# lh3/minigraph

Hardware: NVIDIA H100
Metric: mapped Gbp/s (-cx lr) (higher is better)
Workload: dtype int64/u8 (fp32 chain penalties, bit-exact)

## Files before the change

### include/mgb200.h

```cpp
#ifndef MGB200_H
#define MGB200_H

#include <stdint.h>
#include <stddef.h>

#ifdef __cplusplus
extern "C" {
#endif

#ifndef __GFA_H__
#define __GFA_H__
typedef struct {
	uint64_t v_lv;
	uint32_t w;
	int32_t rank;
	int32_t ov, ow;
	uint64_t link_id:61, strong:1, del:1, comp:1;
} gfa_arc_t;

typedef struct { uint32_t m_aux, l_aux; uint8_t *aux; } gfa_aux_t;

typedef struct gfa_utg_s gfa_utg_t;

typedef struct {
// ... 145 lines not shown
	int64_t n_jobs_side;
	int64_t n_slots;
	double t_pack_ms, t_asm_ms;
	int64_t n_jobs;
	int64_t n_jobs_mid, n_jobs_big;
	int64_t n_reads, n_bases;
	int64_t n_seeds;
	int64_t n_anchors_out;
	int64_t n_chains_out;
	int64_t n_minimizers;
	int64_t out_bytes;
	int64_t n_launches;
	int64_t n_retry;
	uint64_t arena_peak;
	double t_kernel_ms[10];
	uint64_t prof[32];
	double t_lab_ms;
	int64_t n_lab_new;
	int64_t n_lab_big;
	int64_t h2d_bytes;
	double w_gpu_wait_ms;
	double w_slot_wait_ms, w_upload_ms, w_pass_ms, w_redo_ms, w_download_ms;
} mgb_stats_t;

int mgb_test_wfa(const char *ts, int tl, const char *qs, int ql, int64_t max_iter, int step, uint32_t *cigar, int cap, int *score);

#define MGB_TEST_TIER2_CONT 4
int mgb_test_wfa_tier(int tier, int n, const char *ts, const int64_t *t_off, const int32_t *tl, const char *qs, const int64_t *q_off,
					  const int32_t *ql, int64_t *out, uint32_t *cigar, int cap);

int mgb_test_gwfa(const mg_idx_t *gi, int mode, int n, const char *q, const int64_t *q_off, const int32_t *ql, const uint32_t *v0,
// ... 34 lines not shown
```

### minigraph_b200/capi.py

```python
import ctypes as C
import os

MG_M_RMQ = 0x8000
MG_M_CIGAR = 0x4000000
MG_M_PRINT_2ND = 0x2000


class mg128_t(C.Structure):
    _fields_ = [("x", C.c_uint64), ("y", C.c_uint64)]


class mg_idxopt_t(C.Structure):
    _fields_ = [("w", C.c_int), ("k", C.c_int), ("bucket_bits", C.c_int)]


class mg_mapopt_t(C.Structure):
    _fields_ = [
        ("flag", C.c_uint64), ("mini_batch_size", C.c_int64), ("seed", C.c_int), ("max_qlen", C.c_int),
        ("pe_ori", C.c_int), ("occ_max1", C.c_int), ("occ_max1_cap", C.c_int), ("occ_max1_frac", C.c_float),
        ("bw", C.c_int), ("bw_long", C.c_int), ("rmq_size_cap", C.c_int), ("rmq_rescue_size", C.c_int),
        ("rmq_rescue_ratio", C.c_float), ("max_gap_pre", C.c_int), ("max_gap", C.c_int), ("max_gap_ref", C.c_int),
        ("max_frag_len", C.c_int), ("div", C.c_float), ("chn_pen_gap", C.c_float), ("chn_pen_skip", C.c_float),
        ("max_lc_skip", C.c_int), ("max_lc_iter", C.c_int), ("max_gc_skip", C.c_int), ("min_lc_cnt", C.c_int),
        ("min_lc_score", C.c_int), ("min_gc_cnt", C.c_int), ("min_gc_score", C.c_int), ("gdp_max_ed", C.c_int),
# ... 49 lines not shown

class gfa_t(C.Structure):
    _fields_ = [("m_seg", C.c_uint32), ("n_seg", C.c_uint32), ("max_rank", C.c_uint32), ("seg", C.POINTER(gfa_seg_t)),
                ("h_names", C.c_void_p), ("m_sseq", C.c_uint32), ("n_sseq", C.c_uint32),
                ("sseq", C.POINTER(gfa_sseq_t)), ("h_snames", C.c_void_p), ("m_arc", C.c_uint64),
                ("n_arc", C.c_uint64), ("arc", C.c_void_p), ("link_aux", C.c_void_p), ("idx", C.POINTER(C.c_uint64))]


class mgb_stats_t(C.Structure):
    _fields_ = [("t_h2d_ms", C.c_double), ("t_seed_ms", C.c_double), ("t_chain_ms", C.c_double),
                ("t_align_ms", C.c_double), ("t_d2h_ms", C.c_double), ("t_host_ms", C.c_double),
                ("t_wfa_ms", C.c_double), ("t_finish_ms", C.c_double), ("t_dev_span_ms", C.c_double), ("skip1_len", C.c_int64), ("skip2_len", C.c_int64), ("n_jobs_side", C.c_int64), ("n_slots", C.c_int64), ("t_pack_ms", C.c_double), ("t_asm_ms", C.c_double),
                ("n_jobs", C.c_int64), ("n_jobs_mid", C.c_int64), ("n_jobs_big", C.c_int64),
                ("n_reads", C.c_int64), ("n_bases", C.c_int64), ("n_seeds", C.c_int64), ("n_anchors_out", C.c_int64),
                ("n_chains_out", C.c_int64), ("n_minimizers", C.c_int64), ("out_bytes", C.c_int64),
                ("n_launches", C.c_int64), ("n_retry", C.c_int64), ("arena_peak", C.c_uint64), ("t_kernel_ms", C.c_double * 10), ("prof", C.c_uint64 * 32), ("t_lab_ms", C.c_double), ("n_lab_new", C.c_int64), ("n_lab_big", C.c_int64), ("h2d_bytes", C.c_int64),
                ("w_gpu_wait_ms", C.c_double), ("w_slot_wait_ms", C.c_double), ("w_upload_ms", C.c_double), ("w_pass_ms", C.c_double), ("w_redo_ms", C.c_double), ("w_download_ms", C.c_double)]


class mgb_reads_t(C.Structure):
    _fields_ = [("n_reads", C.c_int64), ("n_bases", C.c_int64), ("name", C.POINTER(C.c_char_p)), ("seq", C.POINTER(C.c_char_p)),
                ("len", C.POINTER(C.c_int)), ("block", C.c_void_p)]


KERNEL_NAMES = ["k_seed", "k_chain", "k_gchain", "k_index_sketch", "k_wfa_small", "k_finish", "k_wfa_mid", "k_wfa_big", "k_gwfa", "k_gchain_gen"]
PROF_NAMES = ["wfa_fast_cyc", "wfa_fast_n", "wfa_slow_cyc", "wfa_slow_n", "wfa_max_cyc", "wfa_cells", "wfa_tb_cyc", "gc_dp_cyc", "gc_gen_cyc",
              "gc_post_cyc", "gc_plan_cyc", "fin_cigar_cyc", "fin_ds_cyc", "seed_sketch_cyc", "seed_match_cyc", "seed_sort_cyc", "chain_dp_cyc",
              "chain_onchip_n", "chain_rmq_cyc", "chain_post_cyc", "wfa_mid_cyc", "wfa_mid_n", "gc_gwfa_cyc", "gc_bridge_shortk_cyc", "gc_extra_sort_cyc", "gwfa_max_cyc", "gc_dp_max_cyc", "wfa_handoff_cells", "wfa_handoff_n", "lab_cyc", "lab_n"]
WFA_TIER2_CONT = 4
LCHAIN_DP, LCHAIN_RMQ, LCHAIN_RESCUE = 0, 1, 2
LCHAIN_PATH_DP, LCHAIN_PATH_RMQ_W, LCHAIN_PATH_RMQ_TIE, LCHAIN_PATH_RMQ_CAP = 0, 1, 2, 3


class mgb_lchain_opt_t(C.Structure):
    _fields_ = [(k, C.c_int32) for k in ("max_dist_x", "max_dist_y", "bw", "max_skip", "max_iter", "min_cnt", "min_sc")] + \
               [("pen_gap", C.c_float), ("pen_skip", C.c_float)] + \
               [(k, C.c_int32) for k in ("is_cdna", "n_seg", "max_dist_inner", "cap_rmq_size")]


def bind_mapping_api(lib):
    lib.mg_index.restype = C.POINTER(mg_idx_t)
    lib.mg_index.argtypes = [C.POINTER(gfa_t), C.POINTER(mg_idxopt_t), C.c_int, C.POINTER(mg_mapopt_t)]
    lib.mg_idx_destroy.restype = None
# ... 86 lines not shown
```

### minigraph_b200/csrc/mgb_engine.cu

```cuda
#include <stdio.h>
#include <stdlib.h>
#include <string.h>
#include <math.h>
#include <vector>
#include <algorithm>
#include <string>
#include <chrono>
#include <thread>
#include <mutex>
#include <condition_variable>
#include <functional>
#include <unordered_map>
#include "mgb_hostpool.h"

#include "../../include/mgb200.h"
#include "mgb_galign.cuh"
#include "mgb_gaf.cuh"

#ifndef MGB_HOSTSIM
#include <cuda_runtime.h>
#include "mgb_index.cuh"
#endif

using namespace mgb;
// ... 460 lines not shown
#endif
		}
}
#ifndef MGB_HOSTSIM
__global__ void __launch_bounds__(256) k_unpack(UnpackArgs U)
{
	const int lane = threadIdx.x & 31, warp = (int)((blockIdx.x * blockDim.x + threadIdx.x) >> 5), n_warp = (int)((gridDim.x * blockDim.x) >> 5);
	for (int r = warp; r < U.n_reads; r += n_warp) {
		if (U.pk_off[r] == ~0ULL) continue;
		const int64_t nw = ((int64_t)U.seq_len[r] + 31) >> 5;
		for (int64_t wd = lane; wd < nw; wd += 32) unpack_word(U, r, wd);
	}
}
#endif

struct Mail { Pool pools[16]; unsigned int jobq_n[2], lab_n[2]; unsigned long long prof[32]; unsigned int tier_hist[128]; unsigned long long arena_peak; };
struct MailSrc { const Pool *pools; const unsigned int *jobq_n, *lab_n; const unsigned long long *prof; const unsigned int *tier_hist; const uint64_t *peak; int n_workers; };
#ifndef MGB_HOSTSIM
__global__ void k_mail(MailSrc m, Mail *out)
{
	const int t = threadIdx.x;
	if (t < 16) out->pools[t] = m.pools[t];
	if (t < 2) out->jobq_n[t] = m.jobq_n[t], out->lab_n[t] = m.lab_n? m.lab_n[t] : 0;
	out->prof[t] = m.prof[t];
	for (int i = t; i < 128; i += 32) out->tier_hist[i] = m.tier_hist[i];
	unsigned long long pk = 0;
	for (int i = t; i < m.n_workers; i += 32) pk = m.peak[i] > pk? m.peak[i] : pk;
	for (int o = 16; o > 0; o >>= 1) { const unsigned long long y = __shfl_xor_sync(0xffffffffu, pk, o); pk = y > pk? y : pk; }
	if (t == 0) out->arena_peak = pk;
	__threadfence_system();
}
#endif
MG_HD inline void job_counts(const Pool *pools, int i_gjobs, int i_jobs, unsigned int gjobs_done, unsigned int jobs_done, unsigned int *cnt)
{
	const Pool &pg = pools[i_gjobs], &pj = pools[i_jobs];
	cnt[0] = (unsigned int)((pg.used < pg.cap? pg.used : pg.cap) / sizeof(GwfaJob)) - gjobs_done;
	cnt[1] = (unsigned int)((pj.used < pj.cap? pj.used : pj.cap) / sizeof(WfaJob)) - jobs_done;
}
#ifndef MGB_HOSTSIM
// ... 1189 lines not shown
				if (b1 > b0) memcpy(hout + b0, P.packed + b0, b1 - b0);
#endif
			}
			tm_d2h.stop();
			S.out_bytes = (int64_t)out_bytes;
		}
		if (done) break;
		for (int i = 0; i < N_POOLS; ++i) if (hp[i].used > cap[i]) cap[i] = (hp[i].used * 3 / 2 + 4095) & ~(uint64_t)4095;
		if (attempt == 7) { set_error("output pools kept overflowing"); rc_final = -2; }
	}
	S.t_h2d_ms = tm_h2d.ms(), S.t_seed_ms = tm_seed.ms(), S.t_chain_ms = tm_chain.ms(), S.t_align_ms = tm_align.ms();
	S.t_wfa_ms = tm_wfa.ms(), S.t_finish_ms = tm_fin.ms();
	for (int i = 0; i < 10; ++i) S.t_kernel_ms[i] = tm_k[i].ms();
	S.t_lab_ms = tm_lab.ms();
	S.arena_peak = mail->arena_peak;
	for (int i = 0; i < 32; ++i) S.prof[i] = (uint64_t)mail->prof[i];
	{
		const unsigned int *h = mail->tier_hist;
		int32_t t1 = INT32_MAX;
		for (int b = 0; b < 32 && t1 == INT32_MAX; ++b) { unsigned int in = h[b * 4 + 1], out = h[b * 4 + 2] + h[b * 4 + 3]; if (in + out >= 8 && in < out) t1 = b * 16; }
		unsigned int tot = 0;
		for (int i = 0; i < 128; ++i) tot += h[i];
		if (tot >= 64) { std::lock_guard<std::mutex> lock(M->big_mutex); M->skip1_len = t1; }
		S.skip1_len = L_skip1, S.skip2_len = INT32_MAX;
	}
	if (rc_final < 0) return rc_final;

	double t_asm0 = now_ms();
	S.w_download_ms = t_asm0 - t_host0 - S.w_upload_ms - S.w_pass_ms - S.w_redo_ms - S.w_gpu_wait_ms;
	int first_bad = -1;
	for (int i = 0; i < n_reads; ++i) {
// ... 650 lines not shown
```

### minigraph_b200/csrc/mgb_galign.cuh

```cuda
#pragma once
#include "mgb_pipeline.cuh"
#include "mgb_gchain.cuh"
#include "mgb_wfa_tiers.cuh"
#if defined(MGB_HOSTSIM)
#include <stdio.h>
#include <stdlib.h>
#endif

namespace mgb {

MG_HD inline int cigar_append1(Arena &A, AVec<uint64_t> &c, int32_t op, int32_t len)
{
	if (c.n > 0 && (int32_t)(c.a[c.n - 1] & 0xf) == op) c.a[c.n - 1] += (uint64_t)(int64_t)len << 4;
	else {
		uint64_t x = (uint64_t)(int64_t)len << 4 | (uint64_t)op;
		MGB_TRY(avec_push(A, c, x));
	}
	return 0;
}

MG_HD inline int cigar_append(Arena &A, AVec<uint64_t> &c, int32_t n_cigar, const uint32_t *cigar)
{
	if (n_cigar == 0) return 0;
	MGB_TRY(cigar_append1(A, c, (int32_t)(cigar[0] & 0xf), (int32_t)(cigar[0] >> 4)));
// ... 86 lines not shown
	unsigned long long pt0 = prof_clock();
	int rc;
	int64_t cont_cells = 0;
	if (tier == 1) rc = wfa_smem<WfTier1::W_, WfTier1::MAXLEN_, WfTier1::TBCAP_>(A, smem, tl, tseq, ql, qs, &rst, lane);
	else if (tier == 2 && !t2_long) rc = wfa_smem<WfTier2::W_, WfTier2::MAXLEN_, WfTier2::TBCAP_, true>(A, smem, tl, tseq, ql, qs, &rst, lane, &cont_cells);
	else if (tier == 2) rc = wfa_ring_exact(A, tl, tseq, ql, qs, &rst, lane);
	else rc = wfa_exact(A, tl, tseq, ql, qs, 100000000LL, &rst, lane);
	if (rc < 0) return rc;
	if (lane == 0) {
		unsigned long long dt = prof_clock() - pt0;
		int slot = tier == 1? PROF_WFA_FAST_CYC : tier == 2? PROF_WFA_MID_CYC : PROF_WFA_SLOW_CYC;
		prof_add(c, slot, dt), prof_add(c, slot + 1, 1);
		prof_max(c, PROF_WFA_MAX_CYC, dt << 16 | (unsigned long long)(mlen < 65535? mlen : 65535));
		if (rc == 0) prof_add(c, PROF_WFA_CELLS, (unsigned long long)rst.n_iter);
		if (cont_cells > 0) prof_add(c, PROF_WFA_HANDOFF_N, 1), prof_add(c, PROF_WFA_HANDOFF_CELLS, (unsigned long long)cont_cells);
		if (rc == 0 && explore && c.tier_hist) {
			unsigned int *h = &c.tier_hist[(mlen >> 4 < 31? mlen >> 4 : 31) * 4 + tier];
#if MGB_ON_DEVICE
			atomicAdd(h, 1u);
#else
			++*h;
#endif
		}
	}
	if (rc == 1) {
		if (lane == 0) {
			unsigned int at;
#if MGB_ON_DEVICE
			at = atomicAdd(&c.jobq_n[tier - 1], 1u);
#else
// ... 635 lines not shown
```

### minigraph_b200/csrc/mgb_pipeline.cuh

```cuda
#pragma once
#include "mgb_model.cuh"
#include "mgb_seed.cuh"
#include "mgb_lchain.cuh"
#include "mgb_gclabel.cuh"
#include "mgb_tma.cuh"

namespace mgb {

struct PipeCtx {
	GraphDev g;
	IndexDev ix;
	MapOptDev opt;
	BatchDev b;
	ReadMeta *meta;
	Pool *pool_anchor;     u128 *anchor;
	Pool *pool_minipos;    int32_t *minipos;
	Pool *pool_lchain;     LChain *lchain;
	Pool *pool_out;        char *out;
	Pool *pool_plan;       uint64_t *plan;
	Pool *pool_jobs;       struct WfaJob *jobs;
	Pool *pool_cig;        uint32_t *cig;
	int32_t *jobq[2];      unsigned int *jobq_n;
	Pool *pool_gstate;     char *gstate;
	Pool *pool_gjobs;      struct GwfaJob *gjobs;
	Pool *pool_walk;       int32_t *walk;
	int32_t *rescue_list;  unsigned int *rescue_n;
	LabTab lab;
	unsigned int *next_read;
	unsigned long long *prof;
	int32_t skip1_len;
	unsigned int *tier_hist;
};

enum { PROF_WFA_FAST_CYC = 0, PROF_WFA_FAST_N, PROF_WFA_SLOW_CYC, PROF_WFA_SLOW_N, PROF_WFA_MAX_CYC, PROF_WFA_CELLS, PROF_WFA_TB_CYC,
	   PROF_GC_DP_CYC, PROF_GC_GEN_CYC, PROF_GC_POST_CYC, PROF_GC_PLAN_CYC, PROF_FIN_CIGAR_CYC, PROF_FIN_DS_CYC, PROF_SEED_SKETCH_CYC,
	   PROF_SEED_MATCH_CYC, PROF_SEED_SORT_CYC, PROF_CHAIN_DP_CYC, PROF_CHAIN_BT_CYC, PROF_CHAIN_RMQ_CYC, PROF_CHAIN_POST_CYC, PROF_WFA_MID_CYC, PROF_WFA_MID_N, PROF_GC_GWFA_CYC, PROF_GC_SHORTK_CYC, PROF_GC_EXTRA_CYC, PROF_GWFA_MAX_CYC, PROF_GC_DP_MAX_CYC, PROF_WFA_HANDOFF_CELLS, PROF_WFA_HANDOFF_N, PROF_LAB_CYC, PROF_LAB_N, PROF_N = 32 };

MG_HD inline unsigned long long prof_clock()
{
#if MGB_ON_DEVICE
	return (unsigned long long)clock64();
#else
	return 0;
#endif
}
#if defined(__CUDACC__)
MG_D inline unsigned long long *prof_block() { __shared__ unsigned long long s_prof[PROF_N]; return s_prof; }
MG_D inline bool prof_is_max(int slot) { return slot == PROF_WFA_MAX_CYC || slot == PROF_GWFA_MAX_CYC || slot == PROF_GC_DP_MAX_CYC; }
MG_D inline void prof_block_begin() { if (threadIdx.x < PROF_N) prof_block()[threadIdx.x] = 0; __syncthreads(); }
MG_D inline void prof_block_end(unsigned long long *prof)
{
	__syncthreads();
	if (prof && threadIdx.x < PROF_N) {
		const unsigned long long v = prof_block()[threadIdx.x];
		if (v) { if (prof_is_max((int)threadIdx.x)) atomicMax(&prof[threadIdx.x], v); else atomicAdd(&prof[threadIdx.x], v); }
	}
}
#endif
MG_HD inline void prof_add(const PipeCtx &c, int slot, unsigned long long v)
{
#if MGB_ON_DEVICE
	if (c.prof) atomicAdd(&prof_block()[slot], v);
#else
	if (c.prof) c.prof[slot] += v;
#endif
}
MG_HD inline void prof_max(const PipeCtx &c, int slot, unsigned long long v)
{
#if MGB_ON_DEVICE
	if (c.prof) atomicMax(&prof_block()[slot], v);
// ... 325 lines not shown
```

### minigraph_b200/csrc/mgb_wfa.cuh

```cuda
#pragma once
#include "mgb_common.cuh"

namespace mgb {

static const int32_t WF_NEG_INF = -0x40000000;
static const int WF_X = 4, WF_O1 = 4, WF_E1 = 2, WF_O2 = 15, WF_E2 = 1;
static const int WF_MAX_PEN = 16;
static const int WF_NSLICE = WF_MAX_PEN + 1;
static const int WF_PAD = WF_MAX_PEN + 1;
static const int WF_SEQ_PAD = 16;

#define MGB_WF_MAX(a, b) ((a) >= (b)? (a) : (b))

struct WfResult {
	int32_t s;
	int32_t n_cigar;
	int64_t n_iter;
	uint32_t *cigar;
};


MG_HD inline void wf_stage_seq(char *dst, const char *src, int32_t len, uint8_t sentinel, int lane)
{
	for (int32_t i = lane; i < len; i += MGB_W) dst[i] = src[i];
	for (int32_t i = len + lane; i < len + WF_SEQ_PAD; i += MGB_W) dst[i] = (char)sentinel;
}

MG_HD inline uint32_t wf_ld32u(const char *base, int32_t pos)
{
	const uint32_t *w = (const uint32_t*)base;
	uint32_t lo = w[pos >> 2], hi = w[(pos >> 2) + 1];
	int sh = (pos & 3) << 3;
#if MGB_ON_DEVICE
// ... 21 lines not shown
template<typename TB>
MG_HD inline int wf_traceback(const TB &tb, int32_t n_scores, int32_t tl, const char *ts, int32_t ql, const char *qs, int32_t last_state,
							  uint32_t *cig_store, int64_t max_cigar, int32_t *n_cigar, int64_t *first)
{
	int32_t i = ql - 1, k = tl - 1, s = n_scores - 1, last = last_state;
	int64_t w = max_cigar;
	int32_t cur_op = -1, cur_len = 0;
#define MGB_CIG_PUSH(op_, len_) do { \
		if (cur_op == (op_)) cur_len += (len_); \
		else { \
			if (cur_op >= 0) { if (w <= 0) return MGB_E_INTERNAL; cig_store[--w] = (uint32_t)cur_len << 4 | (uint32_t)cur_op; } \
			cur_op = (op_), cur_len = (len_); \
		} \
	} while (0)
	while (i >= 0 && k >= 0) {
		int32_t k0 = k, x, state, ext;
		if (last == 0) {
			while (i >= 0 && k >= 0 && qs[i] == ts[k]) --i, --k;
			if (k0 - k > 0) MGB_CIG_PUSH(7, k0 - k);
			if (i < 0 || k < 0) break;
		}
		if (s < 0) return MGB_E_INTERNAL;
		x = tb.get(s, i - k);
		if (x < 0) return MGB_E_INTERNAL;
		state = last == 0? x & 7 : last;
		ext = state > 0? x >> (state + 2) & 1 : 0;
		if (state == 0) { MGB_CIG_PUSH(8, 1); --i, --k, s -= WF_X; }
		else if (state == 1) { MGB_CIG_PUSH(1, 1); --i, s -= ext? WF_E1 : WF_O1 + WF_E1; }
		else if (state == 3) { MGB_CIG_PUSH(1, 1); --i, s -= ext? WF_E2 : WF_O2 + WF_E2; }
		else if (state == 2) { MGB_CIG_PUSH(2, 1); --k, s -= ext? WF_E1 : WF_O1 + WF_E1; }
		else if (state == 4) { MGB_CIG_PUSH(2, 1); --k, s -= ext? WF_E2 : WF_O2 + WF_E2; }
		else return MGB_E_INTERNAL;
		last = state > 0 && ext? state : 0;
	}
	if (i >= 0) MGB_CIG_PUSH(1, i + 1);
	else if (k >= 0) MGB_CIG_PUSH(2, k + 1);
	if (cur_op >= 0) { if (w <= 0) return MGB_E_INTERNAL; cig_store[--w] = (uint32_t)cur_len << 4 | (uint32_t)cur_op; }
#undef MGB_CIG_PUSH
// ... 18 lines not shown

template<int W>
MG_HD inline int32_t wfs_col(int32_t d) { return (d + (1 << 20)) & (W - 1); }

struct WfTbSmem {
	const int32_t *row; const uint8_t *x; int32_t n_rows, used;
	MG_HD int32_t get(int32_t s, int32_t d) const
	{
		int32_t lo = row[2 * s], off = row[2 * s + 1];
		int32_t end = s + 1 < n_rows? row[2 * s + 3] : used;
		int32_t j = d - lo;
		return (j < 0 || off + j >= end)? -1 : (int32_t)x[off + j];
	}
};

struct WfTbRow { int32_t lo, hi; uint8_t *x; };
struct WfTbArena {
	const WfTbRow *row;
	MG_HD int32_t get(int32_t s, int32_t d) const
	{
		int32_t j = d - row[s].lo;
		return (j < 0 || j > row[s].hi - row[s].lo)? -1 : (int32_t)row[s].x[j];
	}
};



#define MGB_NL_SYNC(nl) do { if ((nl) > 1) warp_sync(); } while (0)

struct WfSlice {
	int32_t lo, hi;
	int32_t *H, *E1, *F1, *E2, *F2;
};

struct WfState {
	WfSlice sl[WF_NSLICE];
	int32_t *mem;
// ... 154 lines not shown
			wf.lo = wf.hi = seg[sid++].d;
		}
		lo = wf.lo > -tl? wf.lo - 1 : -tl;
		hi = wf.hi < ql? wf.hi + 1 : ql;
		{
			const WfSlice &ft = wf_stripe_add(wf, lo, hi, lane, nl);
			const WfSlice &fx = wf_stripe_get(wf, WF_X);
			const WfSlice &fo1 = wf_stripe_get(wf, WF_O1 + WF_E1);
			const WfSlice &fo2 = wf_stripe_get(wf, WF_O2 + WF_E2);
			const WfSlice &fe1 = wf_stripe_get(wf, WF_E1);
			const WfSlice &fe2 = wf_stripe_get(wf, WF_E2);
			if (nl > 1) MGB_TRY(avec_reserve_w(A, rows, rows.n + 1, lane));
			else MGB_TRY(avec_reserve(A, rows, rows.n + 1));
			uint8_t *x;
			MGB_ALLOC(A, x, uint8_t, hi - lo + 1);
			if (lane == 0) rows.a[rows.n].lo = lo, rows.a[rows.n].hi = hi, rows.a[rows.n].x = x;
			++rows.n;
			uint8_t *ax = x - lo;
			for (int32_t dd = lo + lane; dd <= hi; dd += nl)
				ax[dd] = wf_cell(dd, ft.H, ft.E1, ft.F1, ft.E2, ft.F2, fx.H, fo1.H, fo2.H, fe1.E1, fe1.F1, fe2.E2, fe2.F2);
			MGB_NL_SYNC(nl);
			if (ft.H[lo] >= -1 || ft.E1[lo] >= -1 || ft.F1[lo] >= -1 || ft.E2[lo] >= -1 || ft.F2[lo] >= -1) wf.lo = lo;
			if (ft.H[hi] >= -1 || ft.E1[hi] >= -1 || ft.F1[hi] >= -1 || ft.E2[hi] >= -1 || ft.F2[hi] >= -1) wf.hi = hi;
		}
		if ((wf.s & 0xff) == 0) MGB_TRY(wf_stripe_shrink(wf, tl, ql));
		r->n_iter += hi - lo + 1;
		if (max_iter > 0 && r->n_iter > max_iter) { stopped = 1; break; }
	}
	r->s = stopped? -1 : wf.s;
	if (!stopped) {
		int rc = 0;
// ... 396 lines not shown
```

### minigraph_b200/csrc/mgb_wfa_tiers.cuh

```cuda
#pragma once
#include "mgb_wfa.cuh"

namespace mgb {

#if MGB_ON_DEVICE
MG_D inline uint32_t warp_or_u32(uint32_t x) { return __reduce_or_sync(0xffffffffu, x); }
#elif defined(MGB_SIM_LANES)
inline uint32_t warp_or_u32(uint32_t x) { uint64_t o[32]; sim::exchange(x, o, 15); uint32_t r = 0; for (int i = 0; i < MGB_W; ++i) r |= (uint32_t)o[i]; return r; }
#else
inline uint32_t warp_or_u32(uint32_t x) { return x; }
#endif

#define MGB_OPAQUE(x) asm("" : "+r"(x))

MG_HD inline int32_t wf2_ld(const void *base, int32_t off)
{
	int32_t v = *(const wf_cell_t*)((const char*)base + off);
	MGB_OPAQUE(v);
	return v;
}

#define MGB_WF_CELL_LOAD(S, d_) \
	int32_t h##S, e1##S, e2##S, f1##S, f2##S; \
	uint8_t xz##S; \
// ... 58 lines not shown
	return sc < 0? MGB_WF_RG(1, 0) : sc == 0? MGB_WF_RG(0, 0) : MGB_WF_RG(rows[sc - 1].lo, rows[sc - 1].hi);
}

template<int W>
MG_HD inline int wfa_smem_continue(Arena &A, uint64_t mark, const wf_cell_t *sm, int32_t tl, const char *ts, int32_t ql, const char *qs, WfResult *r,
								   uint32_t *cig_store, int64_t max_cigar, int lane, WfRing &R);

template<int W, int MAXLEN, int TBCAP, bool CONT = false>
MG_HD inline int wfa_smem(Arena &A, int32_t *smem, int32_t tl, const char *ts_g, int32_t ql, const char *qs_g, WfResult *r, int lane, int64_t *cont_cells = 0)
{
	static_assert(!CONT || TBCAP == 0, "the arena ring continues from traceback rows in the arena");
	typedef WfSmemLayout<W, MAXLEN, TBCAP, 17> LY;
	const int HS = 17;
	if (tl > MAXLEN || ql > MAXLEN) return 1;
	if (MAXLEN > 16000) return 1;
	uint64_t mark = A.top;
	wf_cell_t *H = (wf_cell_t*)smem, *E1 = H + HS * W, *F1 = E1 + 3 * W, *E2 = F1 + 3 * W, *F2 = E2 + 2 * W;
	char *ts = (char*)(smem + LY::N_INTS), *qs = ts + LY::SEQ_BYTES;
	int32_t *tb_row = (int32_t*)(qs + LY::SEQ_BYTES);
	uint8_t *tb_x = (uint8_t*)tb_row + LY::TB_ROW_BYTES;
	{
		const uint32_t two = (uint32_t)(uint16_t)(wf_cell_t)WF_NEG_INF16 * 0x10001u;
		uint32_t *cells = (uint32_t*)smem;
		for (int32_t i = lane; i < LY::N_INTS; i += MGB_W) cells[i] = two;
	}
	wf_stage_seq(ts, ts_g, tl, 0xfe, lane);
	wf_stage_seq(qs, qs_g, ql, 0xff, lane);
	r->s = -1, r->n_cigar = 0, r->n_iter = 0, r->cigar = 0;
	uint32_t *cig_store;
	const int64_t max_cigar = (int64_t)tl + ql + 2;
	MGB_ALLOC(A, cig_store, uint32_t, max_cigar);
	uint64_t mark_keep = A.top;
	AVec<WfTbRow> rows;
	avec_init(rows);
	if (TBCAP == 0) MGB_TRY(avec_reserve_w(A, rows, 256, lane));
	int32_t n_rows = 0, tb_used = 0;
	int32_t wlo = 0, whi = 0, last_state = 0, s = 0;
	int64_t n_iter = 0;
	int hs = 0, m3 = 0, m2 = 0;
	const int32_t d_corner = ql - tl;
	int hit = 0, hit_noext = 0;
	warp_sync();
	if (lane == 0) {
		int32_t k0 = -1, k = -1;
		if (!(k0 >= tl || k0 >= ql)) {
			k = wf_extend(ts, qs, k0, 0);
			if (k == tl - 1 && k == ql - 1) hit = 1, hit_noext = (k == k0), k = k0;
		}
		H[wfs_col<W>(0)] = (wf_cell_t)k;
	}
	{
		const uint32_t vb = warp_or_u32((hit? 1u : 0u) | (hit_noext? 2u : 0u));
		hit = vb & 1, hit_noext = vb >> 1 & 1;
	}
	warp_sync();
	for (;;) {
		if (hit) {
			if (hit_noext) {
				int32_t x;
				if (TBCAP > 0) { WfTbSmem t; t.row = tb_row, t.x = tb_x, t.n_rows = n_rows, t.used = tb_used; x = t.get(n_rows - 1, ql - tl); }
				else { WfTbArena t; t.row = rows.a; x = t.get(n_rows - 1, ql - tl); }
				last_state = x & 7;
			}
			break;
		}
		const int32_t lo = wlo > -tl? wlo - 1 : -tl;
		const int32_t hi = whi < ql? whi + 1 : ql;
		const int32_t width = hi - lo + 1;
		if (width + 2 > W || s + 1 >= 255 || (TBCAP > 0 && tb_used + width > TBCAP)) {
			if (CONT && s < 240) {
				WfRing R;
				R.rows = rows, R.n_rows = n_rows, R.wlo = wlo, R.whi = whi, R.s = s, R.hs = hs, R.m3 = m3, R.m2 = m2, R.n_iter = n_iter;
				const int rc = wfa_smem_continue<W>(A, mark_keep, H, tl, ts, ql, qs, r, cig_store, max_cigar, lane, R);
				if (rc < 0) { A.top = mark; return rc; }
				if (r->s < 0) { A.top = mark; return MGB_E_INTERNAL; }
				*cont_cells = r->n_iter - n_iter;
				return 0;
			}
			A.top = mark;
			return 1;
		}
		const int32_t ns = s + 1;
		const int nhs = hs + 1 == 17? 0 : hs + 1, n3 = m3 + 1 == 3? 0 : m3 + 1, n2 = m2 ^ 1;
		uint8_t *ax;
		if (TBCAP > 0) {
			if (lane == 0) tb_row[2 * n_rows] = lo, tb_row[2 * n_rows + 1] = tb_used;
			ax = tb_x + tb_used - lo;
			tb_used += width;
		} else {
			uint8_t *x;
			MGB_ALLOC(A, x, uint8_t, width);
			if (lane == 0) rows.a[n_rows].lo = lo, rows.a[n_rows].hi = hi, rows.a[n_rows].x = x;
			rows.n = n_rows + 1;
			ax = x - lo;
		}
		++n_rows;
		const int r4 = nhs >= WF_X? nhs - WF_X : nhs - WF_X + 17, r6 = nhs >= WF_O1 + WF_E1? nhs - (WF_O1 + WF_E1) : nhs - (WF_O1 + WF_E1) + 17;
		const int r16 = nhs >= WF_O2 + WF_E2? nhs - (WF_O2 + WF_E2) : nhs - (WF_O2 + WF_E2) + 17;
		const int e1slot = n3 >= 2? n3 - 2 : n3 + 1;
		int32_t bHx = r4 * W * 2, bHo1 = r6 * W * 2, bHo2 = r16 * W * 2, bE1 = e1slot * W * 2, bE2 = m2 * W * 2, bnH = nhs * W * 2, bn3 = n3 * W * 2, bn2 = n2 * W * 2;
		MGB_OPAQUE(bHx); MGB_OPAQUE(bHo1); MGB_OPAQUE(bHo2); MGB_OPAQUE(bE1); MGB_OPAQUE(bE2); MGB_OPAQUE(bnH); MGB_OPAQUE(bn3); MGB_OPAQUE(bn2);
		const int32_t colmask2 = 2 * W - 1;
		uint32_t vote = 0;
		for (int32_t d = lo + lane; d <= hi; d += MGB_W) {
			MGB_WF_CELL_LOAD(A, d)
			MGB_WF_CELL_FINISH(A, d)
		}
		vote = warp_or_u32(vote);
		if (vote & 1) wlo = lo;
		if (vote & 2) whi = hi;
		hit = vote >> 2 & 1, hit_noext = vote >> 3 & 1;
		s = ns, hs = nhs, m3 = n3, m2 = n2;
		n_iter += width;
		warp_sync();
	}
	r->n_iter = n_iter;
	r->s = s;
	{
		int rc = 0;
		int32_t n_cig = 0;
		int64_t first = 0;
		if (lane == 0) {
			if (TBCAP > 0) { WfTbSmem t; t.row = tb_row, t.x = tb_x, t.n_rows = n_rows, t.used = tb_used; rc = wf_traceback(t, n_rows, tl, ts, ql, qs, last_state, cig_store, max_cigar, &n_cig, &first); }
			else { WfTbArena t; t.row = rows.a; rc = wf_traceback(t, n_rows, tl, ts, ql, qs, last_state, cig_store, max_cigar, &n_cig, &first); }
		}
		rc = warp_bcast_i32(rc, 0), n_cig = warp_bcast_i32(n_cig, 0), first = (int64_t)warp_bcast_u64((uint64_t)first, 0);
		warp_sync();
		if (rc < 0) { A.top = mark; return rc; }
		r->n_cigar = n_cig, r->cigar = cig_store + first;
	}
	A.top = mark_keep;
	return 0;
}

static const int WF3_NSL = 17 + 3 + 3 + 2 + 2 + 1;
#define MGB_WF2_FILL(need_lo_, need_hi_) do { \
		const int32_t nl_ = (need_lo_), nh_ = (need_hi_); \
		if (fhi < flo || nl_ < flo || nh_ > fhi) { \
			int32_t tlo_ = nl_ - 128 > -tl - 1? nl_ - 128 : -tl - 1, thi_ = nh_ + 128 < ql + 1? nh_ + 128 : ql + 1; \
			if (fhi >= flo) { if (nl_ >= flo) tlo_ = flo; if (nh_ <= fhi) thi_ = fhi; } \
			const int32_t a0_ = tlo_, a1_ = fhi >= flo? flo - 1 : thi_, b0_ = fhi >= flo? fhi + 1 : thi_ + 1, b1_ = thi_; \
			for (int sl_ = 0; sl_ < WF3_NSL; ++sl_) { \
// ... 38 lines not shown
#define MGB_WF_GSET(slot_, v_) (g_all[(slot_)] = (v_))
#endif
	for (;;) {
		if (hit) {
			if (hit_noext) { WfTbArena t; t.row = rows.a; last_state = t.get(n_rows - 1, ql - tl) & 7; }
			break;
		}
		const int32_t lo = wlo > -tl? wlo - 1 : -tl;
		const int32_t hi = whi < ql? whi + 1 : ql;
		const int32_t width = hi - lo + 1;
		const int32_t ns = s + 1;
		const int nhs = hs + 1 == 17? 0 : hs + 1, n3 = m3 + 1 == 3? 0 : m3 + 1, n2 = m2 ^ 1;
		MGB_TRY(avec_reserve_w(A, rows, n_rows + 1, lane));
		uint8_t *x;
		MGB_ALLOC(A, x, uint8_t, width);
		if (lane == 0) rows.a[n_rows].lo = lo, rows.a[n_rows].hi = hi, rows.a[n_rows].x = x;
		rows.n = ++n_rows;
		uint8_t *ax = x - lo;
		const int r4 = nhs >= WF_X? nhs - WF_X : nhs - WF_X + 17, r6 = nhs >= WF_O1 + WF_E1? nhs - (WF_O1 + WF_E1) : nhs - (WF_O1 + WF_E1) + 17;
		const int r16 = nhs >= WF_O2 + WF_E2? nhs - (WF_O2 + WF_E2) : nhs - (WF_O2 + WF_E2) + 17;
		const int e1slot = n3 >= 2? n3 - 2 : n3 + 1;
		MGB_WF2_FILL(lo - 1, hi + 1);
		const uint32_t g16 = MGB_WF_GGET(nhs), g2 = MGB_WF_GGET(nhs >= 3? nhs - 3 : nhs + 14), g1 = MGB_WF_GGET(nhs >= 2? nhs - 2 : nhs + 15);
		MGB_WF2_CLEAN(H + (int64_t)nhs * W, g16);
		MGB_WF2_CLEAN(E1 + (int64_t)n3 * W, g2);
		MGB_WF2_CLEAN(F1 + (int64_t)n3 * W, g2);
		MGB_WF2_CLEAN(E2 + (int64_t)n2 * W, g1);
		MGB_WF2_CLEAN(F2 + (int64_t)n2 * W, g1);
		int32_t bHx = r4 * W * 2, bHo1 = r6 * W * 2, bHo2 = r16 * W * 2, bE1 = e1slot * W * 2, bE2 = m2 * W * 2, bnH = nhs * W * 2, bn3 = n3 * W * 2, bn2 = n2 * W * 2;
		MGB_OPAQUE(bHx); MGB_OPAQUE(bHo1); MGB_OPAQUE(bHo2); MGB_OPAQUE(bE1); MGB_OPAQUE(bE2); MGB_OPAQUE(bnH); MGB_OPAQUE(bn3); MGB_OPAQUE(bn2);
		const int track = ((ns + 16) & 0xff) <= 16;
// ... 29 lines not shown
					if (m) { found = 1; if (pass == 0) nlo = base + ctz32(m); else nhi = base - ctz32(m); break; }
				}
				if (!found) break;
			}
			if (!found) { A.top = mark; return MGB_E_INTERNAL; }
			wlo = nlo, whi = nhi;
		}
		n_iter += width;
		if (max_iter > 0 && n_iter > max_iter) { stopped = 1; break; }
	}
#undef MGB_WF_GGET
#undef MGB_WF_GSET
	r->n_iter = n_iter;
	r->s = stopped? -1 : s;
	if (!stopped) {
		int rc = 0;
		int32_t n_cig = 0;
		int64_t first = 0;
		if (lane == 0) {
			WfTbArena t; t.row = rows.a;
			rc = wf_traceback(t, n_rows, tl, ts, ql, qs, last_state, cig_store, max_cigar, &n_cig, &first);
		}
		rc = warp_bcast_i32(rc, 0), n_cig = warp_bcast_i32(n_cig, 0), first = (int64_t)warp_bcast_u64((uint64_t)first, 0);
		warp_sync();
		if (rc < 0) { A.top = mark; return rc; }
		r->n_cigar = n_cig, r->cigar = cig_store + first;
	}
	A.top = mark;
	return 0;
}

MG_HD inline int wfa_ring_g(Arena &A, int32_t tl, const char *ts, int32_t ql, const char *qs, int64_t max_iter, WfResult *r,
							uint32_t *cig_store, int64_t max_cigar, int lane)
{
	if (tl + ql > 16000 || tl <= 0 || ql <= 0) return 1;
	uint64_t mark = A.top;
	int32_t W = 64;
	while (W < tl + ql + 2) W <<= 1;
	const int32_t mask = W - 1;
// ... 18 lines not shown
		cells[c0] = (wf_cell_t)k;
	}
	{
		const uint32_t vb = warp_or_u32((hit? 1u : 0u) | (hit_noext? 2u : 0u));
		hit = vb & 1, hit_noext = vb >> 1 & 1;
	}
	warp_sync();
	R.cells = cells, R.W = W, R.flo = flo, R.fhi = fhi;
	R.n_rows = 0, R.wlo = R.whi = R.s = 0, R.hs = R.m3 = R.m2 = 0, R.hit = hit, R.hit_noext = hit_noext, R.n_iter = 0;
	return wfa_ring_run(A, mark, tl, ts, ql, qs, max_iter, r, cig_store, max_cigar, lane, R);
}

MG_HD inline bool wf_ring_always_fits(int32_t tl, int32_t ql) { const int64_t n = (int64_t)tl + ql; return (n + 30) * (n + 1) <= 100000000LL; }
MG_HD inline int wfa_ring_exact(Arena &A, int32_t tl, const char *ts_g, int32_t ql, const char *qs_g, WfResult *r, int lane)
{
	r->s = -1, r->n_cigar = 0, r->n_iter = 0, r->cigar = 0;
	uint32_t *cig_store;
	const int64_t max_cigar = (int64_t)tl + ql + 2;
	MGB_ALLOC(A, cig_store, uint32_t, max_cigar);
	const uint64_t mark_keep = A.top;
	char *ts, *qs;
	MGB_ALLOC(A, ts, char, tl + WF_SEQ_PAD + 4);
	MGB_ALLOC(A, qs, char, ql + WF_SEQ_PAD + 4);
	wf_stage_seq(ts, ts_g, tl, 0xfe, lane);
	wf_stage_seq(qs, qs_g, ql, 0xff, lane);
	warp_sync();
	const int rc = wfa_ring_g(A, tl, ts, ql, qs, 100000000LL, r, cig_store, max_cigar, lane);
	if (rc < 0) return rc;
	if (rc != 0 || r->s < 0) return MGB_E_INTERNAL;
	A.top = mark_keep;
	return 0;
}

template<int W>
MG_HD inline int wfa_smem_continue(Arena &A, uint64_t mark, const wf_cell_t *sm, int32_t tl, const char *ts, int32_t ql, const char *qs, WfResult *r,
								   uint32_t *cig_store, int64_t max_cigar, int lane, WfRing &R)
{
	int32_t W2 = 64;
	while (W2 < tl + ql + 2) W2 <<= 1;
	const int32_t mask = W2 - 1;
	MGB_ALLOC(A, R.cells, wf_cell_t, (int64_t)WF3_NSL * W2);
	R.W = W2;
	const int32_t clo = R.rows.a[R.n_rows - 1].lo - 1, chi = R.rows.a[R.n_rows - 1].hi + 1;
	for (int sl = 0; sl < WF3_NSL; ++sl) {
// ... 21 lines not shown
```

Measured before the change: 1.437.

## Add mid-tier WFA phase profiling and speed up traceback and row allocation

Result: no change. 1.428, median of 6 (-0.6%).

```diff
diff --git a/include/mgb200.h b/include/mgb200.h
--- a/include/mgb200.h
+++ b/include/mgb200.h
@@ -183,7 +183,7 @@
 	int64_t n_retry;
 	uint64_t arena_peak;
 	double t_kernel_ms[10];
-	uint64_t prof[32];
+	uint64_t prof[34];
 	double t_lab_ms;
 	int64_t n_lab_new;
 	int64_t n_lab_big;
diff --git a/minigraph_b200/capi.py b/minigraph_b200/capi.py
--- a/minigraph_b200/capi.py
+++ b/minigraph_b200/capi.py
@@ -87,7 +87,7 @@
                 ("n_jobs", C.c_int64), ("n_jobs_mid", C.c_int64), ("n_jobs_big", C.c_int64),
                 ("n_reads", C.c_int64), ("n_bases", C.c_int64), ("n_seeds", C.c_int64), ("n_anchors_out", C.c_int64),
                 ("n_chains_out", C.c_int64), ("n_minimizers", C.c_int64), ("out_bytes", C.c_int64),
-                ("n_launches", C.c_int64), ("n_retry", C.c_int64), ("arena_peak", C.c_uint64), ("t_kernel_ms", C.c_double * 10), ("prof", C.c_uint64 * 32), ("t_lab_ms", C.c_double), ("n_lab_new", C.c_int64), ("n_lab_big", C.c_int64), ("h2d_bytes", C.c_int64),
+                ("n_launches", C.c_int64), ("n_retry", C.c_int64), ("arena_peak", C.c_uint64), ("t_kernel_ms", C.c_double * 10), ("prof", C.c_uint64 * 34), ("t_lab_ms", C.c_double), ("n_lab_new", C.c_int64), ("n_lab_big", C.c_int64), ("h2d_bytes", C.c_int64),
                 ("w_gpu_wait_ms", C.c_double), ("w_slot_wait_ms", C.c_double), ("w_upload_ms", C.c_double), ("w_pass_ms", C.c_double), ("w_redo_ms", C.c_double), ("w_download_ms", C.c_double)]
 
 
@@ -99,7 +99,8 @@
 KERNEL_NAMES = ["k_seed", "k_chain", "k_gchain", "k_index_sketch", "k_wfa_small", "k_finish", "k_wfa_mid", "k_wfa_big", "k_gwfa", "k_gchain_gen"]
 PROF_NAMES = ["wfa_fast_cyc", "wfa_fast_n", "wfa_slow_cyc", "wfa_slow_n", "wfa_max_cyc", "wfa_cells", "wfa_tb_cyc", "gc_dp_cyc", "gc_gen_cyc",
               "gc_post_cyc", "gc_plan_cyc", "fin_cigar_cyc", "fin_ds_cyc", "seed_sketch_cyc", "seed_match_cyc", "seed_sort_cyc", "chain_dp_cyc",
-              "chain_onchip_n", "chain_rmq_cyc", "chain_post_cyc", "wfa_mid_cyc", "wfa_mid_n", "gc_gwfa_cyc", "gc_bridge_shortk_cyc", "gc_extra_sort_cyc", "gwfa_max_cyc", "gc_dp_max_cyc", "wfa_handoff_cells", "wfa_handoff_n", "lab_cyc", "lab_n"]
+              "chain_onchip_n", "chain_rmq_cyc", "chain_post_cyc", "wfa_mid_cyc", "wfa_mid_n", "gc_gwfa_cyc", "gc_bridge_shortk_cyc", "gc_extra_sort_cyc", "gwfa_max_cyc", "gc_dp_max_cyc", "wfa_handoff_cells", "wfa_handoff_n", "lab_cyc", "lab_n",
+              "wfa_mid_setup_cyc", "wfa_mid_loop_cyc", "wfa_mid_ring_cyc"]
 WFA_TIER2_CONT = 4
 LCHAIN_DP, LCHAIN_RMQ, LCHAIN_RESCUE = 0, 1, 2
 LCHAIN_PATH_DP, LCHAIN_PATH_RMQ_W, LCHAIN_PATH_RMQ_TIE, LCHAIN_PATH_RMQ_CAP = 0, 1, 2, 3
diff --git a/minigraph_b200/csrc/mgb_engine.cu b/minigraph_b200/csrc/mgb_engine.cu
--- a/minigraph_b200/csrc/mgb_engine.cu
+++ b/minigraph_b200/csrc/mgb_engine.cu
@@ -498,7 +498,7 @@
 }
 #endif
 
-struct Mail { Pool pools[16]; unsigned int jobq_n[2], lab_n[2]; unsigned long long prof[32]; unsigned int tier_hist[128]; unsigned long long arena_peak; };
+struct Mail { Pool pools[16]; unsigned int jobq_n[2], lab_n[2]; unsigned long long prof[PROF_N]; unsigned int tier_hist[128]; unsigned long long arena_peak; };
 struct MailSrc { const Pool *pools; const unsigned int *jobq_n, *lab_n; const unsigned long long *prof; const unsigned int *tier_hist; const uint64_t *peak; int n_workers; };
 #ifndef MGB_HOSTSIM
 __global__ void k_mail(MailSrc m, Mail *out)
@@ -506,7 +506,7 @@
 	const int t = threadIdx.x;
 	if (t < 16) out->pools[t] = m.pools[t];
 	if (t < 2) out->jobq_n[t] = m.jobq_n[t], out->lab_n[t] = m.lab_n? m.lab_n[t] : 0;
-	out->prof[t] = m.prof[t];
+	for (int i = t; i < PROF_N; i += 32) out->prof[i] = m.prof[i];
 	for (int i = t; i < 128; i += 32) out->tier_hist[i] = m.tier_hist[i];
 	unsigned long long pk = 0;
 	for (int i = t; i < m.n_workers; i += 32) pk = m.peak[i] > pk? m.peak[i] : pk;
@@ -1726,7 +1726,8 @@
 	for (int i = 0; i < 10; ++i) S.t_kernel_ms[i] = tm_k[i].ms();
 	S.t_lab_ms = tm_lab.ms();
 	S.arena_peak = mail->arena_peak;
-	for (int i = 0; i < 32; ++i) S.prof[i] = (uint64_t)mail->prof[i];
+	static_assert(sizeof(S.prof) == sizeof(Mail::prof), "mgb200.h mgb_stats_t.prof has PROF_N counters");
+	for (int i = 0; i < PROF_N; ++i) S.prof[i] = (uint64_t)mail->prof[i];
 	{
 		const unsigned int *h = mail->tier_hist;
 		int32_t t1 = INT32_MAX;
diff --git a/minigraph_b200/csrc/mgb_galign.cuh b/minigraph_b200/csrc/mgb_galign.cuh
--- a/minigraph_b200/csrc/mgb_galign.cuh
+++ b/minigraph_b200/csrc/mgb_galign.cuh
@@ -124,6 +124,8 @@
 		prof_max(c, PROF_WFA_MAX_CYC, dt << 16 | (unsigned long long)(mlen < 65535? mlen : 65535));
 		if (rc == 0) prof_add(c, PROF_WFA_CELLS, (unsigned long long)rst.n_iter);
 		if (cont_cells > 0) prof_add(c, PROF_WFA_HANDOFF_N, 1), prof_add(c, PROF_WFA_HANDOFF_CELLS, (unsigned long long)cont_cells);
+		if (tier == 2) prof_add(c, PROF_WFA_MID_SETUP_CYC, rst.cyc_setup), prof_add(c, PROF_WFA_MID_LOOP_CYC, rst.cyc_loop),
+			prof_add(c, PROF_WFA_MID_RING_CYC, rst.cyc_ring), prof_add(c, PROF_WFA_TB_CYC, rst.cyc_tb);
 		if (rc == 0 && explore && c.tier_hist) {
 			unsigned int *h = &c.tier_hist[(mlen >> 4 < 31? mlen >> 4 : 31) * 4 + tier];
 #if MGB_ON_DEVICE
diff --git a/minigraph_b200/csrc/mgb_pipeline.cuh b/minigraph_b200/csrc/mgb_pipeline.cuh
--- a/minigraph_b200/csrc/mgb_pipeline.cuh
+++ b/minigraph_b200/csrc/mgb_pipeline.cuh
@@ -34,7 +34,8 @@
 
 enum { PROF_WFA_FAST_CYC = 0, PROF_WFA_FAST_N, PROF_WFA_SLOW_CYC, PROF_WFA_SLOW_N, PROF_WFA_MAX_CYC, PROF_WFA_CELLS, PROF_WFA_TB_CYC,
 	   PROF_GC_DP_CYC, PROF_GC_GEN_CYC, PROF_GC_POST_CYC, PROF_GC_PLAN_CYC, PROF_FIN_CIGAR_CYC, PROF_FIN_DS_CYC, PROF_SEED_SKETCH_CYC,
-	   PROF_SEED_MATCH_CYC, PROF_SEED_SORT_CYC, PROF_CHAIN_DP_CYC, PROF_CHAIN_BT_CYC, PROF_CHAIN_RMQ_CYC, PROF_CHAIN_POST_CYC, PROF_WFA_MID_CYC, PROF_WFA_MID_N, PROF_GC_GWFA_CYC, PROF_GC_SHORTK_CYC, PROF_GC_EXTRA_CYC, PROF_GWFA_MAX_CYC, PROF_GC_DP_MAX_CYC, PROF_WFA_HANDOFF_CELLS, PROF_WFA_HANDOFF_N, PROF_LAB_CYC, PROF_LAB_N, PROF_N = 32 };
+	   PROF_SEED_MATCH_CYC, PROF_SEED_SORT_CYC, PROF_CHAIN_DP_CYC, PROF_CHAIN_BT_CYC, PROF_CHAIN_RMQ_CYC, PROF_CHAIN_POST_CYC, PROF_WFA_MID_CYC, PROF_WFA_MID_N, PROF_GC_GWFA_CYC, PROF_GC_SHORTK_CYC, PROF_GC_EXTRA_CYC, PROF_GWFA_MAX_CYC, PROF_GC_DP_MAX_CYC, PROF_WFA_HANDOFF_CELLS, PROF_WFA_HANDOFF_N, PROF_LAB_CYC, PROF_LAB_N,
+	   PROF_WFA_MID_SETUP_CYC, PROF_WFA_MID_LOOP_CYC, PROF_WFA_MID_RING_CYC, PROF_N };
 
 MG_HD inline unsigned long long prof_clock()
 {
@@ -47,13 +48,13 @@
 #if defined(__CUDACC__)
 MG_D inline unsigned long long *prof_block() { __shared__ unsigned long long s_prof[PROF_N]; return s_prof; }
 MG_D inline bool prof_is_max(int slot) { return slot == PROF_WFA_MAX_CYC || slot == PROF_GWFA_MAX_CYC || slot == PROF_GC_DP_MAX_CYC; }
-MG_D inline void prof_block_begin() { if (threadIdx.x < PROF_N) prof_block()[threadIdx.x] = 0; __syncthreads(); }
+MG_D inline void prof_block_begin() { for (int i = threadIdx.x; i < PROF_N; i += blockDim.x) prof_block()[i] = 0; __syncthreads(); }
 MG_D inline void prof_block_end(unsigned long long *prof)
 {
 	__syncthreads();
-	if (prof && threadIdx.x < PROF_N) {
-		const unsigned long long v = prof_block()[threadIdx.x];
-		if (v) { if (prof_is_max((int)threadIdx.x)) atomicMax(&prof[threadIdx.x], v); else atomicAdd(&prof[threadIdx.x], v); }
+	if (prof) for (int i = threadIdx.x; i < PROF_N; i += blockDim.x) {
+		const unsigned long long v = prof_block()[i];
+		if (v) { if (prof_is_max(i)) atomicMax(&prof[i], v); else atomicAdd(&prof[i], v); }
 	}
 }
 #endif
diff --git a/minigraph_b200/csrc/mgb_wfa.cuh b/minigraph_b200/csrc/mgb_wfa.cuh
--- a/minigraph_b200/csrc/mgb_wfa.cuh
+++ b/minigraph_b200/csrc/mgb_wfa.cuh
@@ -17,6 +17,7 @@
 	int32_t n_cigar;
 	int64_t n_iter;
 	uint32_t *cigar;
+	uint32_t cyc_setup, cyc_loop, cyc_ring, cyc_tb;
 };
 
 
@@ -68,14 +69,27 @@
 		} \
 	} while (0)
 	while (i >= 0 && k >= 0) {
-		int32_t k0 = k, x, state, ext;
+		const int32_t x = s >= 0? tb.get(s, i - k) : -1;
+		int32_t k0 = k, state, ext;
 		if (last == 0) {
-			while (i >= 0 && k >= 0 && qs[i] == ts[k]) --i, --k;
+			while (i >= 3 && k >= 3) {
+				const uint32_t y = wf_ld32u(qs, i - 3) ^ wf_ld32u(ts, k - 3);
+				if (y) {
+#if MGB_ON_DEVICE
+					const int32_t n = __clz((int)y) >> 3;
+#else
+					const int32_t n = __builtin_clz(y) >> 3;
+#endif
+					i -= n, k -= n;
+					break;
+				}
+				i -= 4, k -= 4;
+			}
+			if (i < 3 || k < 3) while (i >= 0 && k >= 0 && qs[i] == ts[k]) --i, --k;
 			if (k0 - k > 0) MGB_CIG_PUSH(7, k0 - k);
 			if (i < 0 || k < 0) break;
 		}
 		if (s < 0) return MGB_E_INTERNAL;
-		x = tb.get(s, i - k);
 		if (x < 0) return MGB_E_INTERNAL;
 		state = last == 0? x & 7 : last;
 		ext = state > 0? x >> (state + 2) & 1 : 0;
@@ -124,13 +138,14 @@
 	}
 };
 
-struct WfTbRow { int32_t lo, hi; uint8_t *x; };
+struct alignas(16) WfTbRow { int32_t lo, hi; uint8_t *x; };
 struct WfTbArena {
 	const WfTbRow *row;
 	MG_HD int32_t get(int32_t s, int32_t d) const
 	{
-		int32_t j = d - row[s].lo;
-		return (j < 0 || j > row[s].hi - row[s].lo)? -1 : (int32_t)row[s].x[j];
+		const WfTbRow r = row[s];
+		int32_t j = d - r.lo;
+		return (j < 0 || j > r.hi - r.lo)? -1 : (int32_t)r.x[j];
 	}
 };
 
@@ -315,7 +330,7 @@
 			else MGB_TRY(avec_reserve(A, rows, rows.n + 1));
 			uint8_t *x;
 			MGB_ALLOC(A, x, uint8_t, hi - lo + 1);
-			if (lane == 0) rows.a[rows.n].lo = lo, rows.a[rows.n].hi = hi, rows.a[rows.n].x = x;
+			if (lane == 0) rows.a[rows.n] = WfTbRow{lo, hi, x};
 			++rows.n;
 			uint8_t *ax = x - lo;
 			for (int32_t dd = lo + lane; dd <= hi; dd += nl)
diff --git a/minigraph_b200/csrc/mgb_wfa_tiers.cuh b/minigraph_b200/csrc/mgb_wfa_tiers.cuh
--- a/minigraph_b200/csrc/mgb_wfa_tiers.cuh
+++ b/minigraph_b200/csrc/mgb_wfa_tiers.cuh
@@ -96,6 +96,7 @@
 	const int HS = 17;
 	if (tl > MAXLEN || ql > MAXLEN) return 1;
 	if (MAXLEN > 16000) return 1;
+	const unsigned long long t_setup = prof_clock();
 	uint64_t mark = A.top;
 	wf_cell_t *H = (wf_cell_t*)smem, *E1 = H + HS * W, *F1 = E1 + 3 * W, *E2 = F1 + 3 * W, *F2 = E2 + 2 * W;
 	char *ts = (char*)(smem + LY::N_INTS), *qs = ts + LY::SEQ_BYTES;
@@ -109,6 +110,7 @@
 	wf_stage_seq(ts, ts_g, tl, 0xfe, lane);
 	wf_stage_seq(qs, qs_g, ql, 0xff, lane);
 	r->s = -1, r->n_cigar = 0, r->n_iter = 0, r->cigar = 0;
+	r->cyc_setup = r->cyc_loop = r->cyc_ring = r->cyc_tb = 0;
 	uint32_t *cig_store;
 	const int64_t max_cigar = (int64_t)tl + ql + 2;
 	MGB_ALLOC(A, cig_store, uint32_t, max_cigar);
@@ -117,6 +119,8 @@
 	avec_init(rows);
 	if (TBCAP == 0) MGB_TRY(avec_reserve_w(A, rows, 256, lane));
 	int32_t n_rows = 0, tb_used = 0;
+	uint8_t *tb_blk = 0;
+	int32_t tb_left = 0;
 	int32_t wlo = 0, whi = 0, last_state = 0, s = 0;
 	int64_t n_iter = 0;
 	int hs = 0, m3 = 0, m2 = 0;
@@ -136,6 +140,8 @@
 		hit = vb & 1, hit_noext = vb >> 1 & 1;
 	}
 	warp_sync();
+	const unsigned long long t_loop = prof_clock();
+	r->cyc_setup = (uint32_t)(t_loop - t_setup);
 	for (;;) {
 		if (hit) {
 			if (hit_noext) {
@@ -150,6 +156,8 @@
 		const int32_t hi = whi < ql? whi + 1 : ql;
 		const int32_t width = hi - lo + 1;
 		if (width + 2 > W || s + 1 >= 255 || (TBCAP > 0 && tb_used + width > TBCAP)) {
+			const unsigned long long t_ring = prof_clock();
+			r->cyc_loop = (uint32_t)(t_ring - t_loop);
 			if (CONT && s < 240) {
 				WfRing R;
 				R.rows = rows, R.n_rows = n_rows, R.wlo = wlo, R.whi = whi, R.s = s, R.hs = hs, R.m3 = m3, R.m2 = m2, R.n_iter = n_iter;
@@ -157,6 +165,7 @@
 				if (rc < 0) { A.top = mark; return rc; }
 				if (r->s < 0) { A.top = mark; return MGB_E_INTERNAL; }
 				*cont_cells = r->n_iter - n_iter;
+				r->cyc_ring = (uint32_t)(prof_clock() - t_ring) - r->cyc_tb;
 				return 0;
 			}
 			A.top = mark;
@@ -170,11 +179,11 @@
 			ax = tb_x + tb_used - lo;
 			tb_used += width;
 		} else {
-			uint8_t *x;
-			MGB_ALLOC(A, x, uint8_t, width);
-			if (lane == 0) rows.a[n_rows].lo = lo, rows.a[n_rows].hi = hi, rows.a[n_rows].x = x;
+			if (tb_left < width) { tb_left = 16 * (width + 15); MGB_ALLOC(A, tb_blk, uint8_t, tb_left); }
+			if (lane == 0) rows.a[n_rows] = WfTbRow{lo, hi, tb_blk};
 			rows.n = n_rows + 1;
-			ax = x - lo;
+			ax = tb_blk - lo;
+			tb_blk += width, tb_left -= width;
 		}
 		++n_rows;
 		const int r4 = nhs >= WF_X? nhs - WF_X : nhs - WF_X + 17, r6 = nhs >= WF_O1 + WF_E1? nhs - (WF_O1 + WF_E1) : nhs - (WF_O1 + WF_E1) + 17;
@@ -199,6 +208,8 @@
 	r->n_iter = n_iter;
 	r->s = s;
 	{
+		const unsigned long long t_tb = prof_clock();
+		r->cyc_loop = (uint32_t)(t_tb - t_loop);
 		int rc = 0;
 		int32_t n_cig = 0;
 		int64_t first = 0;
@@ -208,6 +219,7 @@
 		}
 		rc = warp_bcast_i32(rc, 0), n_cig = warp_bcast_i32(n_cig, 0), first = (int64_t)warp_bcast_u64((uint64_t)first, 0);
 		warp_sync();
+		r->cyc_tb = (uint32_t)(prof_clock() - t_tb);
 		if (rc < 0) { A.top = mark; return rc; }
 		r->n_cigar = n_cig, r->cigar = cig_store + first;
 	}
@@ -276,7 +288,7 @@
 		MGB_TRY(avec_reserve_w(A, rows, n_rows + 1, lane));
 		uint8_t *x;
 		MGB_ALLOC(A, x, uint8_t, width);
-		if (lane == 0) rows.a[n_rows].lo = lo, rows.a[n_rows].hi = hi, rows.a[n_rows].x = x;
+		if (lane == 0) rows.a[n_rows] = WfTbRow{lo, hi, x};
 		rows.n = ++n_rows;
 		uint8_t *ax = x - lo;
 		const int r4 = nhs >= WF_X? nhs - WF_X : nhs - WF_X + 17, r6 = nhs >= WF_O1 + WF_E1? nhs - (WF_O1 + WF_E1) : nhs - (WF_O1 + WF_E1) + 17;
@@ -336,6 +348,7 @@
 	r->n_iter = n_iter;
 	r->s = stopped? -1 : s;
 	if (!stopped) {
+		const unsigned long long t_tb = prof_clock();
 		int rc = 0;
 		int32_t n_cig = 0;
 		int64_t first = 0;
@@ -345,6 +358,7 @@
 		}
 		rc = warp_bcast_i32(rc, 0), n_cig = warp_bcast_i32(n_cig, 0), first = (int64_t)warp_bcast_u64((uint64_t)first, 0);
 		warp_sync();
+		r->cyc_tb = (uint32_t)(prof_clock() - t_tb);
 		if (rc < 0) { A.top = mark; return rc; }
 		r->n_cigar = n_cig, r->cigar = cig_store + first;
 	}
@@ -393,7 +407,9 @@
 MG_HD inline bool wf_ring_always_fits(int32_t tl, int32_t ql) { const int64_t n = (int64_t)tl + ql; return (n + 30) * (n + 1) <= 100000000LL; }
 MG_HD inline int wfa_ring_exact(Arena &A, int32_t tl, const char *ts_g, int32_t ql, const char *qs_g, WfResult *r, int lane)
 {
+	const unsigned long long t_ring = prof_clock();
 	r->s = -1, r->n_cigar = 0, r->n_iter = 0, r->cigar = 0;
+	r->cyc_setup = r->cyc_loop = r->cyc_ring = r->cyc_tb = 0;
 	uint32_t *cig_store;
 	const int64_t max_cigar = (int64_t)tl + ql + 2;
 	MGB_ALLOC(A, cig_store, uint32_t, max_cigar);
@@ -407,6 +423,7 @@
 	const int rc = wfa_ring_g(A, tl, ts, ql, qs, 100000000LL, r, cig_store, max_cigar, lane);
 	if (rc < 0) return rc;
 	if (rc != 0 || r->s < 0) return MGB_E_INTERNAL;
+	r->cyc_ring = (uint32_t)(prof_clock() - t_ring) - r->cyc_tb;
 	A.top = mark_keep;
 	return 0;
 }
```
